# harvardinformatics/IMCoalHMM

Hardware: AMD Instinct MI355X
Metric: alignment columns/sec (forward pass), 20-state isolation HMM (higher is better)
Workload: dtype f64

## Files before the change

imcoalhmm_amd/csrc/imcoal_fwd.hip:

```cpp
#include <hip/hip_runtime.h>

#include <algorithm>
#include <array>
#include <cerrno>
#include <climits>
#include <cmath>
#include <cstdint>
#include <cstdio>
#include <cstdlib>
#include <cstring>
#include <list>
#include <atomic>
#include <chrono>
#include <map>
#include <set>
#include <memory>
#include <mutex>
#include <condition_variable>
#include <string>
#include <vector>

#include <sys/stat.h>
#include <unistd.h>

#include "../../include/imcoal_fwd.h"
#include "kernels_plain.hpp"
#include "kernels_stitch.hpp"
#include "kernels_zip.hpp"
#include "kernels_big.hpp"
#include "kernels_zip2.hpp"
#include "kernels_zip3.hpp"
#include "kernels_zip4.hpp"
#include "options_host.hpp"
#include "pair_dict.hpp"
#include "kernels_encode.hpp"
#include "kernels_train.hpp"
#include "kernels_ingest.hpp"
#include "kernels_align.hpp"
#include "kernels_phylip.hpp"
#include "slab_stream.hpp"
#include "plan_host.hpp"
#include "planner_host.hpp"
#include "model_host.hpp"
#include "kernels_model.hpp"
#include "../../include/imcoal_model.h"
#include "kernels_sample.hpp"
#include "../../include/imcoal_sample.h"
#include "obs_io.hpp"
#include "fasta_io.hpp"

static_assert(sizeof(imc::Desc4) == sizeof(int4) && alignof(imc::Desc4) == alignof(int4), "descriptor entries are uploaded as int4");

namespace {

thread_local std::string g_err;
std::mutex g_mu;
std::condition_variable g_cv;

int fail(int code, const std::string &msg)
{
    g_err = msg;
    return code;
}

#define HIP_TRY(expr)                                                                                   \
    do {                                                                                                \
        hipError_t _e = (expr);                                                                         \
        if (_e != hipSuccess)                                                                           \
            return fail(_e == hipErrorOutOfMemory ? IMC_ERR_OOM : IMC_ERR_HIP,                          \
                        std::string(#expr) + ": " + hipGetErrorString(_e));                             \
    } while (0)

using imc::HYBRID_MAX_ALPHABET;
using imc::LDS_BUDGET;
using imc::Z2GRAN;
using imc::round_up;

constexpr size_t STAGE_KERNEL_MAX_BYTES = 1u << 20;

struct GuardRec { hipDeviceptr_t va; size_t va_size; hipMemGenericAllocationHandle_t handle; hipDeviceptr_t map; size_t map_size; };
std::map<void *, GuardRec> &g_guard = *new std::map<void *, GuardRec>();

void dev_free(void *p)
{
    if (!p) return;
    auto it = g_guard.find(p);
    if (it == g_guard.end()) { (void)hipFree(p); return; }
    (void)hipDeviceSynchronize();
    (void)hipMemUnmap(it->second.map, it->second.map_size);
    (void)hipMemRelease(it->second.handle);
    g_guard.erase(it);
}

struct DictDev : imc::TrainedDict {
// ... 1525 lines not shown
        std::vector<std::pair<int, int>> table_runs;
        DevBuf<double> d_Cpack;
        bool rank1 = false;
        std::vector<int> checkpoints;
        std::vector<BigBlock> tail_blocks;
        std::vector<std::pair<uint32_t, uint32_t>> r1_segs;
        DevBuf<BigBlock> d_tail_blocks;
        DevBuf<int> d_r1flag, d_r1at;
        DevBuf<double> d_r1u, d_r1alpha;
    } chain;

    struct Blocked {
        std::vector<Z2Block> blocks;
        DevBuf<Z2Block> d_blocks;
        DevBuf<uint16_t> d_tab_order;
        DevBuf<int> d_tab_lvl;
        std::vector<int> tab_lvl;
        int tab_nlvl = 0;
        DevBuf<int4> d_tab_desc;
        DevBuf<int4> d_tab_desc2;
        std::vector<std::pair<int, int>> tab2;
        DevBuf<int4> d_tab_desc3;
        std::vector<std::pair<int, int>> tab3;
        bool wide_tokens = false;
        bool stream_table = false;
        int n_hot = 0;
        std::vector<uint16_t> hot;
        DevBuf<uint16_t> d_hot;
        imc::PhaseTable phases;
        std::vector<Z2Tail> tails;
        DevBuf<Z2Tail> d_tails;
        DevBuf<double> d_tailX;
        DevBuf<int> d_tailE, d_tail_arrive;
        int tail_stride = 0;
    } blk;
};

struct Level {
    uint32_t n_segs = 0, n_vecs = 0, n_chains = 0;
    DevBuf<uint32_t> d_vec0;
    DevBuf<uint8_t> d_first;
    DevBuf<ChainDesc> d_chains;
    DevBuf<double> d_P;
    DevBuf<int> d_EX, d_EMAX;
};

struct PlanKey {
    std::vector<uint64_t> chunk_ids;
    int N = 0, S = 0, B = 0;
    bool op_mode = false;
    imc::PlanOptions opt;
    bool operator==(const PlanKey &o) const
    {
        return chunk_ids == o.chunk_ids && N == o.N && S == o.S && B == o.B && op_mode == o.op_mode && opt.force_level == o.opt.force_level &&
               imc::same_plan_options(opt, o.opt);
    }
};

struct Plan {
    const PlanKey key;
    KernelChoice *kc = nullptr;
    bool wide = false;
    const int &N = key.N, &S = key.S, &B = key.B;
    const int n_chunks = (int)key.chunk_ids.size();
    uint32_t n_segs = 0, n_vecs = 0;
    std::vector<Group> groups;
    size_t pstride = 0;
    DevBuf<SegDesc> d_segs;
    DevBuf<VecDesc> d_vecs;
    std::vector<Level> levels;
    DevBuf<int32_t> d_final_vec;
    uint64_t chain_steps = 0;
    bool finish_fused = false;
    DevBuf<double> d_params, d_out;
    double *h_params[2] = {nullptr, nullptr};
    hipEvent_t ev_params[2] = {nullptr, nullptr};
    bool ev_used[2] = {false, false};
    int slot = 0;
    double *h_out = nullptr;
    double *h_out_dev = nullptr;
    double *h_params_dev[2] = {nullptr, nullptr};
    hipStream_t last_stream = nullptr;
    int last_slot = 0;
    bool have_last = false;
    bool busy = false;
    hipGraphExec_t graph = nullptr;
    uint64_t calls = 0;
    uint64_t lp[8] = {0, 0, 0, 0, 0, 0, 0, 0};
    std::string kernels;
    explicit Plan(PlanKey k) : key(std::move(k)) {}
    Plan(const Plan &) = delete;
    Plan &operator=(const Plan &) = delete;
    ~Plan()
    {
        if (graph) (void)hipGraphExecDestroy(graph);
        for (int k = 0; k < 2; ++k) {
            if (h_params[k]) (void)hipHostFree(h_params[k]);
            if (ev_params[k]) (void)hipEventDestroy(ev_params[k]);
        }
        if (h_out) (void)hipHostFree(h_out);
    }
};

std::list<std::unique_ptr<Plan>> &g_plans = *new std::list<std::unique_ptr<Plan>>();
constexpr size_t MAX_PLANS = 4;

void wait_all_idle(std::unique_lock<std::mutex> &lk)
// ... 100 lines not shown
void publish_last(const Plan *p)
{
    for (int k = 0; k < 8; ++k) g.last_plan[k] = p->lp[k];
    g.last_kernels = p->kernels;
}

struct DevUpload {
    hipError_t e = hipSuccess;
    template <class T> void alloc(DevBuf<T> &d, size_t bytes)
    {
        if (e == hipSuccess) e = d.alloc(std::max<size_t>(bytes, 16));
    }
    template <class T> void zeroed(DevBuf<T> &d, size_t bytes)
    {
        alloc(d, bytes);
        if (e == hipSuccess) e = hipMemset(d.get(), 0, std::max<size_t>(bytes, 16));
    }
    template <class T, class V> void put(DevBuf<T> &d, const std::vector<V> &h)
    {
        static_assert(sizeof(T) == sizeof(V), "the device buffer holds the host vector's elements");
        alloc(d, h.size() * sizeof(V));
        if (e == hipSuccess && !h.empty()) e = hipMemcpy(d.get(), h.data(), h.size() * sizeof(V), hipMemcpyHostToDevice);
    }
    template <class F> void then(F f)
    {
        if (e == hipSuccess) e = f();
    }
};

struct PlanBuilder {
    const imc_obs *const *chunks = nullptr;
    int n_chunks = 0, N = 0, S = 0, B = 0;
    bool op_mode = false;
    KernelChoice *kc = nullptr;
    bool wide = false;
    bool mfma() const { return kc->use3(opt().blocked_variant) || wide; }
    std::unique_ptr<Plan> p;
    const imc::PlanOptions &opt() const { return p->key.opt; }
    std::vector<int> chunk_group;
    std::vector<SegDesc> segs;
    std::vector<uint8_t> seg_first;
    std::vector<uint32_t> chunk_seg;
    std::vector<VecDesc> vecs;
    std::vector<std::vector<std::pair<uint32_t, uint32_t>>> chunk_units;
    std::vector<uint32_t> chunk_unit, unit_vec0;
    std::vector<uint8_t> unit_first;
    struct HostLevel { std::vector<uint32_t> chunk_seg, vec0; std::vector<uint8_t> first; std::vector<ChainDesc> chains; uint32_t n_vecs; };
    std::vector<HostLevel> hl;
    std::vector<int32_t> final_vec;

    void cut_segments()
    {
        chunk_seg.assign(n_chunks + 1, 0);
        for (int f = 0; f < n_chunks; ++f) {
            chunk_seg[f] = (uint32_t)segs.size();
            const Group &gr = p->groups[chunk_group[f]];
            const size_t L = gr.tokens ? chunks[f]->ntok[gr.level] : chunks[f]->L;
            const uint8_t *base = gr.tokens ? chunks[f]->d_tok[gr.level] : chunks[f]->d_sym;
            if (!L) continue;
            const size_t K0 = (L + gr.seglen - 1) / gr.seglen;
            const size_t sl = round_up((L + K0 - 1) / K0, gr.is_blocked() ? Z2GRAN : 16);
            for (size_t off = 0, k = 0; off < L; off += sl, ++k) {
                const bool wide = gr.tokens ? chunks[f]->wide[gr.level] : chunks[f]->wide_raw;
                const bool fst = k == 0 && !op_mode;
                segs.push_back(SegDesc{base + off * (wide ? 2 : 1), (uint32_t)std::min(sl, L - off),
                                       (fst ? SEG_FIRST : 0u) | (wide ? SEG_WIDE : 0u)});
                seg_first.push_back(fst);
            }
        }
        chunk_seg[n_chunks] = (uint32_t)segs.size();
    }

    int make_units()
    {
        chunk_units.assign(n_chunks, {});
        for (int f = 0; f < n_chunks; ++f) {
            const Group &gr = p->groups[chunk_group[f]];
            const uint32_t step = gr.is_blocked() ? (uint32_t)kc->z4_slots() : 1u;
            for (uint32_t sid = chunk_seg[f]; sid < chunk_seg[f + 1]; sid += step)
                chunk_units[f].push_back({sid, std::min(step, chunk_seg[f + 1] - sid)});
        }
        chunk_unit.assign(n_chunks + 1, 0);
        for (int f = 0; f < n_chunks; ++f) chunk_unit[f + 1] = chunk_unit[f] + (uint32_t)chunk_units[f].size();
        unit_vec0.assign(chunk_unit[n_chunks], 0);
        unit_first.assign(chunk_unit[n_chunks], 0);
        for (Group &gr : p->groups) {
            gr.vec_begin = (uint32_t)vecs.size();
            for (int f : gr.chunks) {
                gr.stream_len += gr.tokens ? chunks[f]->ntok[gr.level] : chunks[f]->L;
                for (size_t u = 0; u < chunk_units[f].size(); ++u) {
                    const uint32_t sid = chunk_units[f][u].first, ns = chunk_units[f][u].second;
                    const uint32_t uid = chunk_unit[f] + (uint32_t)u;
                    const bool fst = seg_first[sid] != 0;
                    unit_first[uid] = fst;
                    unit_vec0[uid] = (uint32_t)vecs.size();
                    const int nv = fst ? 1 : N;
                    for (int c = 0; c < nv; ++c) vecs.push_back(VecDesc{sid, (uint32_t)c});
                    if (gr.is_chain()) { gr.chain.seg_ids.push_back(sid); gr.chain.seg_out.push_back(unit_vec0[uid]); }
                    if (gr.is_blocked()) {
                        std::vector<Z2Block> &blocks = gr.blk.blocks;
                        const bool whole = mfma() && fst && ns == 1 && chunk_units[f].size() == 1;
                        if (whole && !blocks.empty() && blocks.back().first == 2 && blocks.back().n < (uint32_t)kc->z4_slots() &&
                            blocks.back().seg0 + blocks.back().n == sid && blocks.back().out_vec0 + blocks.back().n == unit_vec0[uid])
                            ++blocks.back().n;
                        else
                            blocks.push_back(Z2Block{sid, ns, unit_vec0[uid], whole ? 2u : fst ? 1u : 0u});
                    }
                    for (uint32_t q2 = 0; q2 < ns; ++q2)
                        gr.vsteps += (uint64_t)((seg_first[sid + q2] && !gr.is_blocked()) ? 1 : N) * segs[sid + q2].len;
                }
            }
            gr.n_vecs = (uint32_t)vecs.size() - gr.vec_begin;
        }
        if (p->groups.size() == 1 && p->groups[0].is_blocked() && mfma() && !op_mode && n_chunks > 0) {
            Group::Blocked &bl = p->groups[0].blk;
            bool ok = true;
            size_t most = 0;
            for (int f = 0; f < n_chunks; ++f) {
                ok = ok && !chunk_units[f].empty() && chunk_units[f].size() <= (size_t)kc->z4_slots();
// ... 165 lines not shown
                u.zeroed(ch.d_r1flag, nrec * 4);
                u.zeroed(ch.d_r1at, nrec * 4);
                u.alloc(ch.d_r1u, nrec * kc->NP * 8);
                u.alloc(ch.d_r1alpha, nrec * kc->NP * 8);
            }
        }
        u.alloc(q->d_params, (size_t)B * q->pstride * 8);
        u.alloc(q->d_out, (size_t)B * std::max(n_chunks, 1) * 8);
        for (int k = 0; k < 2; ++k) {
            u.then([&] { return hipHostMalloc((void **)&q->h_params[k], (size_t)B * q->pstride * 8, hipHostMallocMapped); });
            u.then([&] { return hipHostGetDevicePointer((void **)&q->h_params_dev[k], q->h_params[k], 0); });
            u.then([&] { return hipEventCreateWithFlags(&q->ev_params[k], hipEventDisableTiming); });
        }
        u.then([&] { return hipHostMalloc((void **)&q->h_out, (size_t)B * std::max(n_chunks, 1) * 8, hipHostMallocMapped); });
        u.then([&] { return hipHostGetDevicePointer((void **)&q->h_out_dev, q->h_out, 0); });
        if (u.e != hipSuccess)
            return fail(u.e == hipErrorOutOfMemory ? IMC_ERR_OOM : IMC_ERR_HIP,
                        std::string("plan allocation: ") + hipGetErrorString(u.e));
        g_plans.push_front(std::move(p));
        *out = q;
        return IMC_OK;
    }
};

void gather_facts(const imc_obs *const *chunks, int n_chunks, std::vector<imc::ChunkFacts> &cf, std::vector<imc::DictFacts> &df,
                  std::vector<std::shared_ptr<DictDev>> &dict_of)
{
    cf.resize(n_chunks);
    for (int f = 0; f < n_chunks; ++f) {
        const imc_obs *o = chunks[f];
        imc::ChunkFacts &c = cf[f];
        c.L = o->L; c.nsym = o->nsym; c.wide_raw = o->wide_raw;
        if (o->dict) {
            c.dict = (int)(std::find(dict_of.begin(), dict_of.end(), o->dict) - dict_of.begin());
            if (c.dict == (int)dict_of.size()) { dict_of.push_back(o->dict); df.push_back(imc::DictFacts{&o->dict->depth}); }
        }
        for (int l = 0; l < imc::kNumLevels; ++l)
            c.level[l] = imc::ChunkFacts::Level{o->d_tok[l] != nullptr, o->wide[l], o->ntok[l], o->alphabet[l], &o->tok_count[l]};
    }
}

int build_plan(const imc_obs *const *chunks, int n_chunks, int N, int S, int B, bool op_mode, Plan **out)
{
    PlanKey key;
    key.chunk_ids.reserve(n_chunks);
    for (int f = 0; f < n_chunks; ++f) key.chunk_ids.push_back(chunks[f]->id);
    key.N = N; key.S = S; key.B = B; key.op_mode = op_mode;
    static_cast<imc::Options &>(key.opt) = g.opt;
    key.opt.cus = g.cus;
    const char *force_level = std::getenv("IMC_FORCE_LEVEL");
    key.opt.force_level = force_level ? std::atoi(force_level) : -1;
    key.opt.debug = std::getenv("IMC_DEBUG") != nullptr;
    key.opt.debug_levels = std::getenv("IMC_DEBUG_LEVELS") != nullptr;
    const imc::PlanOptions &opt = key.opt;
    for (auto it = g_plans.begin(); it != g_plans.end(); ++it) {
        if ((*it)->key == key) {
            g_plans.splice(g_plans.begin(), g_plans, it);
            *out = g_plans.front().get();
            return IMC_OK;
        }
    }
    std::vector<imc::ChunkFacts> cf;
    std::vector<imc::DictFacts> df;
    std::vector<std::shared_ptr<DictDev>> dict_of;
    gather_facts(chunks, n_chunks, cf, df, dict_of);

    KernelChoice *kc = choose_kernel(N, imc::prefer_gemm(opt, cf, N, S));
    if (!kc) return fail(IMC_ERR_ARG, "N exceeds the largest built kernel (" + std::to_string(IMC_MAX_N) + ")");
    if (kc->R == 0 && (kc->G == 7 || kc->G == 9) && kc + 1 < kChoices + sizeof(kChoices) / sizeof(kChoices[0]) &&
        imc::next_shape_hands_off(opt, *kc, *(kc + 1), cf, S, B))
        kc = kc + 1;
    imc::PlanDecision dec = imc::decide_groups(opt, *kc, false, cf, df, N, S, B, op_mode);
    bool wide = false;
    KernelChoice *kw = (N > 24 && N <= 32) ? choose_kernel(N, false) : nullptr;
    if (kw && kw->wide_blocked && opt.wide_blocked != 0 && opt.compression == 1 && opt.kernel_pref == 0 && n_chunks > 0) {
        imc::PlanDecision wdec = imc::decide_groups(opt, *kw, true, cf, df, N, S, B, op_mode);
        if (imc::wide_plan_wins(opt, dec, kc->R == 0, wdec, cf, N)) {
            dec = std::move(wdec);
            kc = kw;
            wide = true;
        }
    }
    PlanBuilder pb;
    pb.chunks = chunks; pb.n_chunks = n_chunks; pb.N = N; pb.S = S; pb.B = B; pb.op_mode = op_mode; pb.kc = kc; pb.wide = wide;
    pb.p = std::make_unique<Plan>(std::move(key));
    pb.p->kc = kc; pb.p->wide = wide;
    pb.chunk_group = std::move(dec.chunk_group);
    for (imc::GroupDecision &gd : dec.groups) {
        Group gr;
        gr.kind = gd.kind; gr.tokens = gd.tokens; gr.level = gd.level; gr.A = gd.A;
        if (gd.dict >= 0) gr.dict = dict_of[gd.dict];
        gr.chunks = std::move(gd.chunks);
        gr.seglen = gd.seglen; gr.model_us = gd.model_us; gr.model_tab_us = gd.model_tab_us;
        gr.blk.wide_tokens = gd.wide_tokens;
        gr.chain.rank1 = gd.rank1; gr.chain.checkpoints = std::move(gd.checkpoints);
        pb.p->groups.push_back(std::move(gr));
    }
    pb.cut_segments();
    if (int rc = pb.make_units()) return rc;
    pb.make_hierarchy();
    return pb.upload(out);
}

int check_args(const imc_obs *const *chunks, int n_chunks, int B, int N, int S, const double *pis,
               const double *Ts, const double *Es)
{
// ... 237 lines not shown
                                   (const int4 *)gr.blk.d_tab_desc3.get(), lc.first, lc.second, staged);
            else
                hipLaunchKernelGGL(kc->zip4_level3, grid, dim3(Z4L3_WAVES * 64), kc->zip4_level3_lds(0), stream, ba,
                                   (const int4 *)gr.blk.d_tab_desc3.get(), lc.first, lc.second, none);
            head = false;
            HIP_TRY(hipGetLastError());
        }
    } else if (opt.table_pairs && gr.blk.d_tab_desc2 && kc->zip4_level2) {
        const size_t split_max = opt.table_split_max >= 0 ? (size_t)opt.table_split_max : (size_t)4 * opt.cus;
        for (const auto &lc : gr.blk.tab2) {
            if (opt.table_split && (size_t)lc.second * B <= split_max) {
                if (head)
                    hipLaunchKernelGGL(kc->zip4_level2_split_first, dim3((unsigned)(lc.second + Z4_SPLIT_WAVES_FIRST - 1) / Z4_SPLIT_WAVES_FIRST, (unsigned)B),
                                       dim3(Z4_SPLIT_WAVES_FIRST * 64), p->pstride * 8, stream, ba,
                                       (const int4 *)gr.blk.d_tab_desc2.get(), lc.first, lc.second, staged);
                else
                    hipLaunchKernelGGL(kc->zip4_level2_split, dim3((unsigned)(lc.second + Z4_SPLIT_WAVES - 1) / Z4_SPLIT_WAVES, (unsigned)B),
                                       dim3(Z4_SPLIT_WAVES * 64), 0, stream, ba,
                                       (const int4 *)gr.blk.d_tab_desc2.get(), lc.first, lc.second, none);
                split_used = true;
            } else if (head)
                hipLaunchKernelGGL(kc->zip4_level2_first, dim3((unsigned)(lc.second + 3) / 4, (unsigned)B), dim3(64),
                                   p->pstride * 8, stream, ba,
                                   (const int4 *)gr.blk.d_tab_desc2.get(), lc.first, lc.second, staged);
            else
                hipLaunchKernelGGL(kc->zip4_level2, dim3((unsigned)(lc.second + 3) / 4, (unsigned)B), dim3(64), 0, stream, ba,
                                   (const int4 *)gr.blk.d_tab_desc2.get(), lc.first, lc.second, none);
            head = false;
            HIP_TRY(hipGetLastError());
        }
    } else
        for (int d = 0; d < gr.blk.tab_nlvl; ++d) {
            const int first = gr.blk.tab_lvl[d], count = gr.blk.tab_lvl[d + 1] - first;
            hipLaunchKernelGGL(kc->zip4_level, dim3((unsigned)(count + 3) / 4, (unsigned)B), dim3(64), 0, stream, ba, first, count);
            HIP_TRY(hipGetLastError());
        }
    return IMC_OK;
}

int Launch::zip4(const Group &gr)
{
    BigArgs ba = blocked_args(gr);
    if (int rc = z4_table(gr, ba)) return rc;
    void (*scan)(BigArgs) = gr.blk.stream_table ? (gr.blk.wide_tokens ? kc->zip4sw : kc->zip4s) : (gr.blk.wide_tokens ? kc->zip4w : kc->zip4);
    if (int rc = allow_lds_budget(scan)) return rc;
    if (int rc = mark_a()) return rc;
    dim3 scan_grid(ba.n_group_segs, (unsigned)B);
    if (opt.xcd_affine && B > 1) {
        const imc::PhaseTable &t = gr.blk.phases;
        ba.n_phases = t.n_phases;
        for (int k = 0; k < t.n_phases; ++k) { ba.ph_begin[k] = t.ph_begin[k]; ba.ph_first[k] = t.ph_first[k]; ba.ph_sets[k] = t.ph_sets[k]; }
        scan_grid = dim3((unsigned)t.grid);
    }
    hipLaunchKernelGGL(scan, scan_grid, dim3(kc->z4_waves * 64), kc->zip4_lds(gr.A, gr.blk.n_hot), stream, ba);
    note(std::string("k_zpropagate4<") + std::to_string(kc->NP / 4) + (gr.blk.wide_tokens ? ",16" : "") + (gr.blk.stream_table ? ",streamed>" : ">") + stream_tag(gr));
    account(gr);
    HIP_TRY(hipGetLastError());
    return IMC_OK;
}

int Launch::zip32(const Group &gr)
{
    BigArgs ba = blocked_args(gr);
    const bool v3 = kc->use3(opt.blocked_variant);
    void (*scan)(BigArgs) = v3 ? kc->zip3 : kc->zip2;
    if (int rc = allow_lds_budget(scan)) return rc;
    size_t lds3 = kc->blocked_lds(gr.A, opt.blocked_variant);
    if (direct_params) { ba.params_src = p->h_params_dev[p->slot]; lds3 = ((lds3 + 15) & ~(size_t)15) + p->pstride * 8; }
    hipLaunchKernelGGL(scan, dim3(ba.n_group_segs, (unsigned)p->B), dim3(Z2WAVES * 64), lds3, stream, ba);
    note(std::string(v3 ? "k_zpropagate3<" : "k_zpropagate2<") + std::to_string(kc->NP / 4) + ">" + stream_tag(gr));
    account(gr);
    HIP_TRY(hipGetLastError());
    return IMC_OK;
}


int Launch::zpropagate(const Group &gr)
{
    const size_t lds = kc->zip_lds(gr.A);
    if (int rc = allow_lds_budget(kc->zip)) return rc;
    const uint32_t vpb = (uint32_t)(ZWAVES * kc->VPW);
    dim3 grid((gr.n_vecs + vpb - 1) / vpb, (unsigned)p->B);
    hipLaunchKernelGGL(kc->zip, grid, dim3(ZWAVES * 64), lds, stream, prop_args(p, gr));
    note("k_zpropagate<" + std::to_string(kc->R) + "," + std::to_string(kc->G) + ">" + stream_tag(gr));
    account(gr);
    HIP_TRY(hipGetLastError());
    return IMC_OK;
}

int Launch::propagate(const Group &gr)
{
    const uint32_t vpb = (uint32_t)(WPB * kc->VPW);
    dim3 grid((gr.n_vecs + vpb - 1) / vpb, (unsigned)p->B);
    const size_t lds = ((size_t)WPB * kc->VPW * kc->NP + (size_t)p->S * kc->NP) * 8;
    if (lds > LDS_BUDGET) return fail(IMC_ERR_ARG, "emission table (S x N) too large for LDS");
    if (lds > 48 * 1024)
        if (int rc = allow_lds_budget(kc->plain)) return rc;
    hipLaunchKernelGGL(kc->plain, grid, dim3(WPB * 64), lds, stream, prop_args(p, gr));
    note("k_propagate<" + std::to_string(kc->R) + "," + std::to_string(kc->G) + ">" + stream_tag(gr));
    account(gr);
    HIP_TRY(hipGetLastError());
    return IMC_OK;
}


int Launch::stitch() const
// ... 1315 lines not shown
```

imcoalhmm_amd/csrc/kernels_big.hpp:

```cpp
#pragma once
#include "kernels_plain.hpp"

typedef double v4f64 __attribute__((ext_vector_type(4)));

struct Z2Block {
    uint32_t seg0, n;
    uint32_t out_vec0;
    uint32_t first;
};

struct Z2Tail { uint32_t chunk, unit, n_units, pad; };

struct BigArgs {
    const SegDesc *segs;
    const uint32_t *seg_ids;
    const uint32_t *seg_vec0;
    const Z2Block *blocks;
    uint32_t n_group_segs;
    uint32_t n_vecs_total;
    int N, S, A;
    const double *params;
    const double *params_src;
    size_t pstride;
    int PP;
    const uint16_t *tok_left, *tok_right;
    double *Ctab;
    int *cex;
    double *P;
    int *EX;
    int phase;
    int t_from, t_to;
    int *r1flag;
    int *r1at;
    double *r1u, *r1alpha;
    uint32_t n_segs;
    const uint16_t *tab_order;
    const int *tab_lvl;
    int tab_nlvl;
    const uint16_t *hot;
    int n_hot;
    const int4 *tab_desc;
    double *Cpack;
    int TS;
    const Z2Tail *tail;
    double *tailX;
    int *tailE;
    int *tail_arrive;
    double *tail_out;
    int tail_stride, n_chunks;
    int n_phases, ph_begin[4], ph_first[4], ph_sets[4];
};


template <int NT>
struct BigLds {
    static constexpr int NP = 16 * NT;
    static constexpr int APS = 18;
    static constexpr int BPS = NP + 4;
    static constexpr int A_DOUBLES = NP * APS, B_DOUBLES = 16 * BPS;
    static constexpr size_t bytes = (size_t)2 * (A_DOUBLES + B_DOUBLES) * 8;
};

template <int NT, int TC = NT>
__device__ __forceinline__ void big_gemm(const double *__restrict__ A, const double *__restrict__ B, int row0, int col0,
                                         int tid, double *lds, v4f64 (&acc)[1][TC])
{
    using L = BigLds<NT>;
    constexpr int NP = 16 * NT, TR = 1, THREADS = NT * 64;
    constexpr int APS = L::APS, BPS = L::BPS;
    const int lane = tid & 63, lm = lane & 15, lg = lane >> 4;
    const int e0 = tid, e1 = tid + THREADS;
    const int ar0 = e0 >> 3, ac0 = e0 & 7, ar1 = e1 >> 3, ac1 = e1 & 7;
    const int br0 = e0 / (NP / 2), bc0 = e0 - br0 * (NP / 2), br1 = e1 / (NP / 2), bc1 = e1 - br1 * (NP / 2);
    const double *gA0 = A + (size_t)ar0 * NP + 2 * ac0, *gA1 = A + (size_t)ar1 * NP + 2 * ac1;
    const double *gB0 = B + (size_t)br0 * NP + 2 * bc0, *gB1 = B + (size_t)br1 * NP + 2 * bc1;
    const int lA0 = ar0 * APS + 2 * ac0, lA1 = ar1 * APS + 2 * ac1;
    const int lB0 = L::A_DOUBLES + br0 * BPS + 2 * bc0, lB1 = L::A_DOUBLES + br1 * BPS + 2 * bc1;
    double2 sa0, sa1, sb0, sb1;
#define BIG_FETCH(kb_)                                                                 \
    do {                                                                               \
        sa0 = *reinterpret_cast<const double2 *>(gA0 + (kb_) * 16);                    \
        sa1 = *reinterpret_cast<const double2 *>(gA1 + (kb_) * 16);                    \
        sb0 = *reinterpret_cast<const double2 *>(gB0 + (size_t)(kb_) * 16 * NP);       \
        sb1 = *reinterpret_cast<const double2 *>(gB1 + (size_t)(kb_) * 16 * NP);       \
    } while (0)
#define BIG_STAGE(buf_)                                                                \
    do {                                                                               \
        double *base_ = lds + (buf_) * (L::A_DOUBLES + L::B_DOUBLES);                  \
        *reinterpret_cast<double2 *>(base_ + lA0) = sa0;                               \
        *reinterpret_cast<double2 *>(base_ + lA1) = sa1;                               \
        *reinterpret_cast<double2 *>(base_ + lB0) = sb0;                               \
        *reinterpret_cast<double2 *>(base_ + lB1) = sb1;                               \
    } while (0)
#pragma unroll
    for (int tr = 0; tr < TR; ++tr)
#pragma unroll
        for (int tc = 0; tc < TC; ++tc) acc[tr][tc] = v4f64{0.0, 0.0, 0.0, 0.0};
    BIG_FETCH(0);
    BIG_STAGE(0);
    __syncthreads();
#pragma unroll 1
    for (int kb = 0; kb < NP / 16; ++kb) {
        const int buf = kb & 1;
// ... 828 lines not shown
```

imcoalhmm_amd/csrc/kernels_zip4.hpp:

```cpp
#pragma once
#include "kernels_zip3.hpp"

template <int NT>
struct Zip4Shape {
    static constexpr int WAVES = NT <= 6 ? Z2WAVES : 4;
    static constexpr int SLOTS = WAVES * 4;
    static constexpr bool SLOT_MAP = NT <= 6;
};

template <int NT>
struct Zip4Geom {
    using G3 = Zip3Geom<NT>;
    static constexpr int TOK = G3::TOK;
    static constexpr int SLOTS = Zip4Shape<NT>::SLOTS;
    static constexpr int MAPS = Zip4Shape<NT>::SLOT_MAP ? 2 : 1;
    static constexpr int slots(int H) { return (H + 1 > SLOTS + 1 ? H + 1 : SLOTS + 1); }
    static constexpr size_t lds_bytes(int A, int H) { return (size_t)slots(H) * TOK * 8 + (size_t)(MAPS * (A + 2) + 64) * 4 + 16; }
    static constexpr int max_hot(int A, size_t budget)
    {
        const size_t fixed = (size_t)(MAPS * (A + 2) + 64) * 4 + 16;
        const size_t n = budget > fixed ? (budget - fixed) / ((size_t)TOK * 8) : 0;
        return n > 1 ? (int)n - 1 : 0;
    }
};
// ... 543 lines not shown
    const double *Gt = a.Ctab + (size_t)b * (a.A + 1) * TOK;
    const int *Gc = a.cex + (size_t)b * (a.A + 1);
    const int IDENT = a.A;
    const double *Gi = Gt + (size_t)IDENT * TOK;

    Z4_STAMP(0);
    for (int z = tid; z <= a.A; z += THREADS) { cex[z] = Gc[z]; if constexpr (SLOT_MAP) slot_of[z] = -1; }
    if constexpr (HYB) {
        __syncthreads();
        for (int k = tid; k <= H; k += THREADS) slot_of[k < H ? (int)a.hot[k] : IDENT] = k;
        for (int idx = tid; idx < (H + 1) * (TOK / 2); idx += THREADS) {
            const int k = idx / (TOK / 2), w = idx - k * (TOK / 2);
            const int z = k < H ? (int)a.hot[k] : IDENT;
            reinterpret_cast<double2 *>(C + (size_t)k * TOK)[w] = reinterpret_cast<const double2 *>(Gt + (size_t)z * TOK)[w];
        }
    }
    __syncthreads();

    Z4_STAMP(1);
    const int lane = tid & 63;
    const int q = lane >> 4, bq = (lane >> 2) & 3, r = lane & 3;
    const int lo = (q * 4 + r) * Geo::NTE, lx = q * 4 + r;
    const Z2Block blk = a.blocks[bx];
    const int slot = (tid >> 6) * 4 + bq;
    const bool valid = slot < (int)blk.n;
    const uint32_t seg = blk.seg0 + (valid ? slot : ((slot & ~3) < (int)blk.n ? (slot & ~3) : 0));
    const SegDesc sd = a.segs[seg];
    const int len = valid ? (int)sd.len : 0;
    const bool first = (sd.first & SEG_FIRST) != 0;
    const uint8_t *tokp = sd.obs;
    typedef const __attribute__((address_space(1))) uint8_t *gptr;
    typedef uint32_t u32x4 __attribute__((ext_vector_type(4)));
    typedef const __attribute__((address_space(1))) u32x4 *gptr4;
    typedef const __attribute__((address_space(1))) uint32_t *gptr1;
    const gptr tokg = (gptr)tokp;

    double P[NT][NT], Q[NT][NT];
    {
        const int tok0 = (valid && first) ? seg_token(tokp, WIDE, 0) : 0;
#pragma unroll
        for (int K = 0; K < NT; ++K)
#pragma unroll
            for (int J = 0; J < NT; ++J) {
                const int i = 4 * K + q, c = 4 * J + r;
                double v;
                if (first) v = (c == 0 && i < a.N) ? pi_p[i] * Etg[(size_t)tok0 * a.PP + i] : 0.0;
                else v = (i == c && i < a.N) ? 1.0 : 0.0;
                P[K][J] = valid ? v : 0.0;
            }
    }
    int ex = 0;
    const int maxlen = wave_max_i32(len);
    const int nfull = maxlen == 0 ? 0 : wave_min_i32(valid ? len / RESCALE_EVERY : INT_MAX);

    constexpr int RING = (!HYB && NT <= 4) ? 2 : 1;
    constexpr int ROWS = NT == 8 ? 4 : NT;
    double al[NT] = {}, pre[RING][ROWS][NT];
#pragma unroll
    for (int d = 0; d < RING; ++d)
#pragma unroll
        for (int I = 0; I < ROWS; ++I)
#pragma unroll
            for (int K = 0; K < NT; ++K) pre[d][I][K] = 0.0;
    auto mk = [&](int tok) __attribute__((always_inline)) {
        Z4Tok t;
        t.s = HYB ? slot_of[tok] : -1;
        t.ce = cex[tok];
        t.tok = tok;
        return t;
    };
    auto prime = [&](const Z4Tok &c, const Z4Tok &c1) __attribute__((always_inline)) {
        if constexpr (HYB) zip3_load_row<NT>(al, C + (size_t)max(c.s, 0) * TOK, 0, lo, lx);
        const double *Gc0 = c.s < 0 ? Gt + (size_t)c.tok * TOK : Gi;
#pragma unroll
        for (int I = 0; I < ROWS; ++I) zip4_load_row_global<NT>(pre[0][I], Gc0, I, lo, lx);
        if constexpr (RING == 2) {
            const double *Gc1 = Gt + (size_t)c1.tok * TOK;
#pragma unroll
            for (int I = 0; I < ROWS; ++I) zip4_load_row_global<NT>(pre[1][I], Gc1, I, lo, lx);
        }
    };
    auto two_steps = [&](const Z4Tok &t0, const Z4Tok &t1, const Z4Tok &tn, const Z4Tok &tn1) __attribute__((always_inline)) {
        if constexpr (RING == 2) {
            zip4_step<NT, HYB, ROWS>(P, Q, C, Gt, Gi, t0, t1, tn, al, pre[0], lo, lx);
            zip4_step<NT, HYB, ROWS>(Q, P, C, Gt, Gi, t1, tn, tn1, al, pre[1], lo, lx);
        } else {
            zip4_step<NT, HYB, ROWS>(P, Q, C, Gt, Gi, t0, t1, t1, al, pre[0], lo, lx);
            zip4_step<NT, HYB, ROWS>(Q, P, C, Gt, Gi, t1, tn, tn, al, pre[0], lo, lx);
        }
        ex += t0.ce + t1.ce;
    };
    constexpr int PER = WIDE ? 8 : 16;
    auto masked_run = [&](int bi, int u0, int n) __attribute__((always_inline)) {
        uint4 ob = make_uint4(0u, 0u, 0u, 0u);
        if (bi * RESCALE_EVERY + u0 < len) {
            const u32x4 v = *(gptr4)(tokg + ((size_t)bi * RESCALE_EVERY + u0) * TB);
            ob = make_uint4(v.x, v.y, v.z, v.w);
        }
        const int live = len - bi * RESCALE_EVERY - u0;
        const int dead0 = (first && bi == 0 && u0 == 0) ? 0 : -1;
        const unsigned long long lo64 = (unsigned long long)ob.y << 32 | ob.x, hi64 = (unsigned long long)ob.w << 32 | ob.z;
        auto tok_of = [&](int v) __attribute__((always_inline)) {
            const unsigned long long h = v < PER / 2 ? lo64 : hi64;
            const int tk = WIDE ? (int)((h >> (16 * (v & 3))) & 0xffffull) : (int)((h >> (8 * (v & 7))) & 0xffull);
            return (v < live && v != dead0 && v < PER) ? tk : IDENT;
        };
        Z4Tok c0 = mk(tok_of(0)), c1 = mk(tok_of(1));
        prime(c0, c1);
#pragma unroll 1
        for (int v = 0; v < n; v += 2) {
            const Z4Tok c2 = mk(tok_of(v + 2)), c3 = mk(tok_of(v + 3));
            two_steps(c0, c1, c2, c3);
            c0 = c2;
            c1 = c3;
        }
    };
    auto masked_block = [&](int bi, int npos) __attribute__((always_inline)) {
#pragma unroll 1
        for (int u0 = 0; u0 < npos; u0 += PER) masked_run(bi, u0, min(PER, npos - u0));
        zip3_rescale<NT>(P, ex);
    };
    if (nfull == 0 && maxlen > 0) masked_block(0, min(RESCALE_EVERY, (maxlen + 1) & ~1));
    Z4_STAMP(2);
    if (nfull > 0) {
        constexpr int NW = 4 * TB;
        constexpr uint32_t TM = WIDE ? 0xffffu : 0xffu;
        auto load_words = [&](int bi, uint32_t (&w)[NW]) __attribute__((always_inline)) {
            gptr4 src = (gptr4)(tokg + (size_t)bi * RESCALE_EVERY * TB);
            const u32x4 x = src[0];
            w[0] = x.x; w[1] = x.y; w[2] = x.z; w[3] = x.w;
            if constexpr (WIDE) {
                const u32x4 y = src[1];
                w[4] = y.x; w[5] = y.y; w[6] = y.z; w[7] = y.w;
            }
        };
        uint32_t cw[NW];
        load_words(0, cw);
        Z4Tok c0 = mk(first ? IDENT : (int)(cw[0] & TM));
        prime(c0, mk(WIDE ? (int)(cw[0] >> 16) : (int)((cw[0] >> 8) & TM)));
        for (int bi = 0; bi < nfull; ++bi) {
            const bool more = bi + 1 < nfull;
            const int bn = more ? bi + 1 : bi;
            const uint32_t nfirst = *(gptr1)(tokg + (size_t)bn * RESCALE_EVERY * TB);
#pragma unroll
            for (int g4 = 0; g4 < 4; ++g4) {
                int t1, t2, t3, t4;
                if constexpr (WIDE) {
                    const uint32_t wa = cw[0], wb = cw[1];
#pragma unroll
                    for (int k = 0; k + 2 < NW; ++k) cw[k] = cw[k + 2];
                    t1 = (int)(wa >> 16); t2 = (int)(wb & TM); t3 = (int)(wb >> 16);
                } else {
                    const uint32_t wa = cw[0];
#pragma unroll
                    for (int k = 0; k + 1 < NW; ++k) cw[k] = cw[k + 1];
                    t1 = (int)((wa >> 8) & TM); t2 = (int)((wa >> 16) & TM); t3 = (int)(wa >> 24);
                }
                t4 = g4 < 3 ? (int)(cw[0] & TM) : more ? (int)(nfirst & TM) : IDENT;
                const uint32_t w5 = g4 < 3 ? cw[0] : nfirst;
                const int t5 = (g4 < 3 || more) ? (WIDE ? (int)(w5 >> 16) : (int)((w5 >> 8) & TM)) : IDENT;
                if (g4 == 3) load_words(bn, cw);
                const Z4Tok c1 = mk(t1), c2 = mk(t2), c3 = mk(t3);
                two_steps(c0, c1, c2, c3);
                const Z4Tok c4 = mk(t4), c5 = mk(t5);
                two_steps(c2, c3, c4, c5);
                c0 = c4;
            }
            zip3_rescale<NT>(P, ex);
        }
    }
    Z4_STAMP(3);
    for (int bi = max(1, nfull); bi * RESCALE_EVERY < maxlen; ++bi)
        masked_block(bi, min(RESCALE_EVERY, (maxlen - bi * RESCALE_EVERY + 1) & ~1));
    zip3_rescale<NT>(P, ex);
    Z4_STAMP(4);
#ifdef IMC_Z4_TIMING
    if ((threadIdx.x & 63) == 0 && blockIdx.x < 1024 && blockIdx.y == 0) g_z4_dbg[1024 * 8 + blockIdx.x * 8 + (threadIdx.x >> 6)] = wall_clock64();
#endif

    if (blk.first == 2) {
        if (valid && r == 0) {
            const size_t gvp = (size_t)b * a.n_vecs_total + blk.out_vec0 + slot;
#pragma unroll
            for (int K = 0; K < NT; ++K)
                if (4 * K + q < a.N) a.P[gvp * NP + 4 * K + q] = P[K][0];
            if (q == 0) a.EX[gvp] = ex;
        }
        return;
    }

    zip3_fold<NT, HYB, true, SLOTS>(P, ex, C, xex, (int)blk.n, slot, tid >> 6, lo, lx);

    Z4_STAMP(5);
#ifdef IMC_Z4_TIMING
    if (threadIdx.x == 0 && blockIdx.x < 1024 && blockIdx.y == 0) g_z4_dbg[blockIdx.x * 8 + 7] = (long long)nfull * 1000000 + maxlen;
#endif
    if (slot == 0) {
        const size_t gv = (size_t)b * a.n_vecs_total + blk.out_vec0;
        double *Pout = a.P + gv * NP;
        if (blk.first) {
            if (r == 0) {
#pragma unroll
                for (int K = 0; K < NT; ++K)
                    if (4 * K + q < a.N) Pout[4 * K + q] = P[K][0];
            }
            if (q == 0 && r == 0) a.EX[gv] = ex;
        } else {
#pragma unroll
            for (int K = 0; K < NT; ++K)
#pragma unroll
                for (int J = 0; J < NT; ++J) {
                    const int i = 4 * K + q, c = 4 * J + r;
                    if (i < a.N && c < a.N) Pout[(size_t)i * NP + c] = P[K][J];
                }
            if (q == 0) {
#pragma unroll
                for (int J = 0; J < NT; ++J)
                    if (4 * J + r < a.N) a.EX[gv + 4 * J + r] = ex;
            }
        }
    }
    if (a.tail) zip3_tail<NT, SLOTS>(a, P, ex, C, xex, b, bx, slot, lo, lx);
}
```

imcoalhmm_amd/csrc/planner_host.hpp:

```cpp
#pragma once

#include <algorithm>
#include <cmath>
#include <cstddef>
#include <cstdint>
#include <cstdio>
#include <functional>
#include <map>
#include <set>
#include <utility>
#include <vector>

#include "options_host.hpp"
#include "pair_dict.hpp"
#include "plan_host.hpp"

namespace imc {

constexpr double Z4_STREAM_MAX_BYTES = 32.0e6;
constexpr size_t LDS_BUDGET = 160 * 1024 - 1024;
constexpr size_t CTAB_BUDGET = (size_t)24 << 30;
#ifndef IMC_HYBRID_MAX_ALPHABET
#define IMC_HYBRID_MAX_ALPHABET 4096
#endif
constexpr int HYBRID_MAX_ALPHABET = IMC_HYBRID_MAX_ALPHABET;
constexpr size_t Z2GRAN = 4;
constexpr size_t R1_MIN_SEGLEN = 1024;
constexpr size_t R1_MIN_HEAD = 256;
constexpr double R1_HEAD_COLUMNS = 65536.0;
constexpr double R1_HEAD_MIN_COLUMNS = 8192.0;
constexpr int R1_MAX_ROUNDS = 24;
constexpr double R1_DENSE_COLUMNS = 1.0e5;

enum class GroupKind {
    ColumnVector,
    TokenVector,
    BlockedLds,
    BlockedGlobal,
    GemmChain,
    MatVecChain,
};

struct PlanOptions : Options {
    int cus = 256;
    int force_level = -1;
    bool debug = false;
    bool debug_levels = false;
};

struct KernelFacts {
    int R = 0, G = 0, NP = 0, VPW = 0, minw = 1;
    int zwaves = 0;
    int big_nslab = 0;
    size_t big_lds = 0;
    int tok_doubles = 0;
    int z4_waves = 8;
    bool wide_blocked = false;
    bool has_zip2 = false, has_zip3 = false, has_zip4 = false, has_zip4s = false, has_level2 = false;
    size_t (*zip_lds)(int) = nullptr;
    size_t (*zip2_lds)(int) = nullptr;
    size_t (*zip3_lds)(int) = nullptr;
    size_t (*zip4_lds)(int, int) = nullptr;
    int (*zip4_max_hot)(int, size_t) = nullptr;
    int z4_slots() const { return z4_waves * 4; }
    bool use3(int blocked_variant) const { return has_zip3 && blocked_variant >= 3; }
    size_t blocked_lds(int A, int blocked_variant) const { return use3(blocked_variant) ? zip3_lds(A) : zip2_lds(A); }
};

struct ChunkFacts {
    size_t L = 0;
    int nsym = 0;
    bool wide_raw = false;
    int dict = -1;
    struct Level {
        bool stream = false;
        bool wide = false;
        size_t ntok = 0;
        int alphabet = 0;
        const std::vector<uint32_t> *tok_count = nullptr;
        const std::vector<uint32_t> &counts() const
        {
            static const std::vector<uint32_t> none;
            return tok_count ? *tok_count : none;
        }
    } level[kNumLevels];
};

struct DictFacts {
    const std::vector<int> *depth = nullptr;
};

struct GroupDecision {
    bool tokens = false;
    int level = -1, A = 0;
    int dict = -1;
    std::vector<int> chunks;
    GroupKind kind = GroupKind::ColumnVector;
    size_t seglen = 0;
    bool wide_tokens = false;
    bool rank1 = false;
// ... 482 lines not shown
```

Before: 400.2 billion.

## Balance segment cuts across CUs and pipeline the uniform tail block in zip4

Adds a host-side balanced cutter that uses spare workgroup slots in the last dispatch round to split long chunks into more, shorter segments. Within each workgroup it alternates two segment lengths across the slot halves. In the zip4 scan kernel, when every lane shares the same length and the remainder after the full rescale blocks is even, the tail is run as a pipelined continuation of the token stream instead of the masked block path. Both are on by default and can be turned off with environment variables. The risks are uneven per-lane lengths breaking the uniform-length assumption, and extra segment joins adding stitch work.

```diff
diff --git a/imcoalhmm_amd/csrc/cut_host.hpp b/imcoalhmm_amd/csrc/cut_host.hpp
--- /dev/null
+++ b/imcoalhmm_amd/csrc/cut_host.hpp
@@ -0,0 +1,79 @@
+#pragma once
+
+#include <algorithm>
+#include <cstddef>
+#include <cstdint>
+#include <vector>
+
+namespace imc {
+
+struct ChunkCut {
+    uint32_t a = 0, b = 0;
+    uint32_t workgroups = 0;
+    bool balanced = false;
+};
+
+inline size_t equal_seglen(size_t L, size_t seglen, size_t gran)
+{
+    const size_t K0 = (L + seglen - 1) / seglen;
+    return ((L + K0 - 1) / K0 + gran - 1) / gran * gran;
+}
+
+inline void cut_lengths(const ChunkCut &c, size_t L, int slots, std::vector<uint32_t> &out)
+{
+    out.clear();
+    for (size_t off = 0, k = 0; off < L; ++k) {
+        const size_t len = std::min<size_t>((int)(k % (size_t)slots) < slots / 2 ? c.a : c.b, L - off);
+        out.push_back((uint32_t)len);
+        off += len;
+    }
+}
+
+inline std::vector<ChunkCut> balanced_cut(const std::vector<size_t> &tokens, size_t seglen, int slots, int B, int cus, size_t gran,
+                                          size_t keep_within = 0)
+{
+    const size_t n = tokens.size(), half = (size_t)slots / 2;
+    std::vector<ChunkCut> cut(n);
+    std::vector<size_t> W(n, 0);
+    size_t total = 0, run = 0;
+    for (size_t f = 0; f < n; ++f) {
+        const size_t L = tokens[f];
+        if (!L) continue;
+        const size_t sl = equal_seglen(L, seglen, gran), nseg = (L + sl - 1) / sl;
+        cut[f].a = cut[f].b = (uint32_t)sl;
+        W[f] = (nseg + slots - 1) / slots;
+        cut[f].workgroups = (uint32_t)W[f];
+        if (nseg == 1) { if (run++ % (size_t)slots == 0) ++total; }
+        else { run = 0; total += W[f]; }
+    }
+    if (B < 1 || cus < 1 || half == 0 || slots % 2) return cut;
+    auto sum_len = [&](size_t L, size_t w) { return ((L + half * w - 1) / (half * w) + gran - 1) / gran * gran; };
+    const size_t wgs = total * (size_t)B, rounds = (wgs + cus - 1) / (size_t)cus;
+    std::vector<size_t> Wn = W;
+    for (size_t spare = (rounds * (size_t)cus - wgs) / (size_t)B; spare > 0; --spare) {
+        size_t best = n;
+        for (size_t f = 0; f < n; ++f) {
+            if (W[f] < 2 || sum_len(tokens[f], Wn[f] + 1) < 32) continue;
+            if (W[f] <= keep_within && Wn[f] + 1 > keep_within) continue;
+            if (best == n || tokens[f] * Wn[best] > tokens[best] * Wn[f]) best = f;
+        }
+        if (best == n) break;
+        ++Wn[best];
+    }
+    for (size_t f = 0; f < n; ++f) {
+        if (W[f] < 2) continue;
+        const size_t L = tokens[f], T = sum_len(L, Wn[f]);
+        if (T < 32) continue;
+        size_t a = T / 2 / 16 * 16;
+        if (a < 16 || T - 2 * a >= 16) a = T / 2 / gran * gran;
+        const size_t b = T - a;
+        if (a == b && (Wn[f] == W[f] || a == cut[f].a)) continue;
+        cut[f].a = (uint32_t)a;
+        cut[f].b = (uint32_t)b;
+        cut[f].workgroups = (uint32_t)((L + half * T - 1) / (half * T));
+        cut[f].balanced = true;
+    }
+    return cut;
+}
+
+}
diff --git a/imcoalhmm_amd/csrc/imcoal_fwd.hip b/imcoalhmm_amd/csrc/imcoal_fwd.hip
--- a/imcoalhmm_amd/csrc/imcoal_fwd.hip
+++ b/imcoalhmm_amd/csrc/imcoal_fwd.hip
@@ -40,6 +40,7 @@
 #include "kernels_phylip.hpp"
 #include "slab_stream.hpp"
 #include "plan_host.hpp"
+#include "cut_host.hpp"
 #include "planner_host.hpp"
 #include "model_host.hpp"
 #include "kernels_model.hpp"
@@ -1671,7 +1672,7 @@
     imc::PlanOptions opt;
     bool operator==(const PlanKey &o) const
     {
-        return chunk_ids == o.chunk_ids && N == o.N && S == o.S && B == o.B && op_mode == o.op_mode && opt.force_level == o.opt.force_level &&
+        return chunk_ids == o.chunk_ids && N == o.N && S == o.S && B == o.B && op_mode == o.op_mode && opt.force_level == o.opt.force_level && opt.balanced_cut == o.opt.balanced_cut && opt.tail_pipe == o.opt.tail_pipe &&
                imc::same_plan_options(opt, o.opt);
     }
 };
@@ -1878,19 +1879,37 @@
     void cut_segments()
     {
         chunk_seg.assign(n_chunks + 1, 0);
+        auto stream_len = [&](int f) { const Group &gr = p->groups[chunk_group[f]]; return gr.tokens ? chunks[f]->ntok[gr.level] : chunks[f]->L; };
+        std::vector<imc::ChunkCut> balanced(n_chunks);
+        for (const Group &gr : p->groups) {
+            if (!opt().balanced_cut || !gr.global_table() || wide || kc->z4_waves != 8 || op_mode || opt().seg_override) continue;
+            std::vector<size_t> lens;
+            bool packs = false;
+            for (int f : gr.chunks) {
+                lens.push_back(stream_len(f));
+                packs = packs || (lens.back() && lens.back() <= imc::equal_seglen(lens.back(), gr.seglen, Z2GRAN));
+            }
+            if (packs && p->groups.size() > 1) continue;
+            const size_t keep = opt().fuse_tail == 0 ? 0 : opt().fuse_tail == 2 ? (size_t)kc->z4_slots() : 4;
+            const std::vector<imc::ChunkCut> cut = imc::balanced_cut(lens, gr.seglen, kc->z4_slots(), B, opt().cus, Z2GRAN, keep);
+            for (size_t k = 0; k < gr.chunks.size(); ++k) balanced[gr.chunks[k]] = cut[k];
+        }
+        std::vector<uint32_t> lens;
         for (int f = 0; f < n_chunks; ++f) {
             chunk_seg[f] = (uint32_t)segs.size();
             const Group &gr = p->groups[chunk_group[f]];
-            const size_t L = gr.tokens ? chunks[f]->ntok[gr.level] : chunks[f]->L;
+            const size_t L = stream_len(f);
             const uint8_t *base = gr.tokens ? chunks[f]->d_tok[gr.level] : chunks[f]->d_sym;
             if (!L) continue;
-            const size_t K0 = (L + gr.seglen - 1) / gr.seglen;
-            const size_t sl = round_up((L + K0 - 1) / K0, gr.is_blocked() ? Z2GRAN : 16);
-            for (size_t off = 0, k = 0; off < L; off += sl, ++k) {
+            imc::ChunkCut cut = balanced[f];
+            if (!cut.balanced)
+                cut.a = cut.b = (uint32_t)imc::equal_seglen(L, gr.seglen, gr.is_blocked() ? Z2GRAN : 16);
+            imc::cut_lengths(cut, L, kc->z4_slots(), lens);
+            size_t off = 0;
+            for (size_t k = 0; k < lens.size(); off += lens[k], ++k) {
                 const bool wide = gr.tokens ? chunks[f]->wide[gr.level] : chunks[f]->wide_raw;
                 const bool fst = k == 0 && !op_mode;
-                segs.push_back(SegDesc{base + off * (wide ? 2 : 1), (uint32_t)std::min(sl, L - off),
-                                       (fst ? SEG_FIRST : 0u) | (wide ? SEG_WIDE : 0u)});
+                segs.push_back(SegDesc{base + off * (wide ? 2 : 1), lens[k], (fst ? SEG_FIRST : 0u) | (wide ? SEG_WIDE : 0u)});
                 seg_first.push_back(fst);
             }
         }
@@ -2162,6 +2181,10 @@
     key.opt.force_level = force_level ? std::atoi(force_level) : -1;
     key.opt.debug = std::getenv("IMC_DEBUG") != nullptr;
     key.opt.debug_levels = std::getenv("IMC_DEBUG_LEVELS") != nullptr;
+    const char *balanced_cut = std::getenv("IMC_BALANCED_CUT");
+    key.opt.balanced_cut = !balanced_cut || std::atoi(balanced_cut) != 0;
+    const char *tail_pipe = std::getenv("IMC_TAIL_PIPE");
+    key.opt.tail_pipe = !tail_pipe || std::atoi(tail_pipe) != 0;
     const imc::PlanOptions &opt = key.opt;
     for (auto it = g_plans.begin(); it != g_plans.end(); ++it) {
         if ((*it)->key == key) {
@@ -2505,6 +2528,7 @@
         for (int k = 0; k < t.n_phases; ++k) { ba.ph_begin[k] = t.ph_begin[k]; ba.ph_first[k] = t.ph_first[k]; ba.ph_sets[k] = t.ph_sets[k]; }
         scan_grid = dim3((unsigned)t.grid);
     }
+    ba.z4_tail_pipe = opt.tail_pipe ? 1 : 0;
     hipLaunchKernelGGL(scan, scan_grid, dim3(kc->z4_waves * 64), kc->zip4_lds(gr.A, gr.blk.n_hot), stream, ba);
     note(std::string("k_zpropagate4<") + std::to_string(kc->NP / 4) + (gr.blk.wide_tokens ? ",16" : "") + (gr.blk.stream_table ? ",streamed>" : ">") + stream_tag(gr));
     account(gr);
diff --git a/imcoalhmm_amd/csrc/kernels_big.hpp b/imcoalhmm_amd/csrc/kernels_big.hpp
--- a/imcoalhmm_amd/csrc/kernels_big.hpp
+++ b/imcoalhmm_amd/csrc/kernels_big.hpp
@@ -49,6 +49,7 @@
     double *tail_out;
     int tail_stride, n_chunks;
     int n_phases, ph_begin[4], ph_first[4], ph_sets[4];
+    int z4_tail_pipe;
 };
 
 
diff --git a/imcoalhmm_amd/csrc/kernels_zip4.hpp b/imcoalhmm_amd/csrc/kernels_zip4.hpp
--- a/imcoalhmm_amd/csrc/kernels_zip4.hpp
+++ b/imcoalhmm_amd/csrc/kernels_zip4.hpp
@@ -619,6 +619,8 @@
     int ex = 0;
     const int maxlen = wave_max_i32(len);
     const int nfull = maxlen == 0 ? 0 : wave_min_i32(valid ? len / RESCALE_EVERY : INT_MAX);
+    const int rem = maxlen - nfull * RESCALE_EVERY;
+    const bool piped = a.z4_tail_pipe != 0 && nfull > 0 && rem > 0 && (rem & 1) == 0 && wave_min_i32(valid ? len : INT_MAX) == maxlen;
 
     constexpr int RING = (!HYB && NT <= 4) ? 2 : 1;
     constexpr int ROWS = NT == 8 ? 4 : NT;
@@ -692,21 +694,21 @@
     if (nfull > 0) {
         constexpr int NW = 4 * TB;
         constexpr uint32_t TM = WIDE ? 0xffffu : 0xffu;
-        auto load_words = [&](int bi, uint32_t (&w)[NW]) __attribute__((always_inline)) {
+        auto load_words = [&](int bi, uint32_t (&w)[NW], bool second) __attribute__((always_inline)) {
             gptr4 src = (gptr4)(tokg + (size_t)bi * RESCALE_EVERY * TB);
             const u32x4 x = src[0];
             w[0] = x.x; w[1] = x.y; w[2] = x.z; w[3] = x.w;
             if constexpr (WIDE) {
-                const u32x4 y = src[1];
+                const u32x4 y = src[second ? 1 : 0];
                 w[4] = y.x; w[5] = y.y; w[6] = y.z; w[7] = y.w;
             }
         };
         uint32_t cw[NW];
-        load_words(0, cw);
+        load_words(0, cw, true);
         Z4Tok c0 = mk(first ? IDENT : (int)(cw[0] & TM));
         prime(c0, mk(WIDE ? (int)(cw[0] >> 16) : (int)((cw[0] >> 8) & TM)));
         for (int bi = 0; bi < nfull; ++bi) {
-            const bool more = bi + 1 < nfull;
+            const bool more = bi + 1 < nfull || piped;
             const int bn = more ? bi + 1 : bi;
             const uint32_t nfirst = *(gptr1)(tokg + (size_t)bn * RESCALE_EVERY * TB);
 #pragma unroll
@@ -726,7 +728,7 @@
                 t4 = g4 < 3 ? (int)(cw[0] & TM) : more ? (int)(nfirst & TM) : IDENT;
                 const uint32_t w5 = g4 < 3 ? cw[0] : nfirst;
                 const int t5 = (g4 < 3 || more) ? (WIDE ? (int)(w5 >> 16) : (int)((w5 >> 8) & TM)) : IDENT;
-                if (g4 == 3) load_words(bn, cw);
+                if (g4 == 3) load_words(bn, cw, bi + 1 < nfull || !piped || rem > 8);
                 const Z4Tok c1 = mk(t1), c2 = mk(t2), c3 = mk(t3);
                 two_steps(c0, c1, c2, c3);
                 const Z4Tok c4 = mk(t4), c5 = mk(t5);
@@ -735,9 +737,29 @@
             }
             zip3_rescale<NT>(P, ex);
         }
+        if (piped) {
+#pragma unroll 1
+            for (int v = 0; v < rem; v += 2) {
+                int t1, t2, t3;
+                if constexpr (WIDE) {
+                    t1 = (int)(cw[0] >> 16); t2 = (int)(cw[1] & TM); t3 = (int)(cw[1] >> 16);
+#pragma unroll
+                    for (int k = 0; k + 1 < NW; ++k) cw[k] = cw[k + 1];
+                } else {
+                    t1 = (int)((cw[0] >> 8) & TM); t2 = (int)((cw[0] >> 16) & TM); t3 = (int)(cw[0] >> 24);
+#pragma unroll
+                    for (int k = 0; k + 1 < NW; ++k) cw[k] = cw[k] >> 16 | cw[k + 1] << 16;
+                    cw[NW - 1] >>= 16;
+                }
+                const Z4Tok c1 = mk(t1), c2 = mk(v + 2 < rem ? t2 : IDENT), c3 = mk(v + 3 < rem ? t3 : IDENT);
+                two_steps(c0, c1, c2, c3);
+                c0 = c2;
+            }
+            zip3_rescale<NT>(P, ex);
+        }
     }
     Z4_STAMP(3);
-    for (int bi = max(1, nfull); bi * RESCALE_EVERY < maxlen; ++bi)
+    for (int bi = piped ? INT_MAX / RESCALE_EVERY : max(1, nfull); bi * RESCALE_EVERY < maxlen; ++bi)
         masked_block(bi, min(RESCALE_EVERY, (maxlen - bi * RESCALE_EVERY + 1) & ~1));
     zip3_rescale<NT>(P, ex);
     Z4_STAMP(4);
diff --git a/imcoalhmm_amd/csrc/planner_host.hpp b/imcoalhmm_amd/csrc/planner_host.hpp
--- a/imcoalhmm_amd/csrc/planner_host.hpp
+++ b/imcoalhmm_amd/csrc/planner_host.hpp
@@ -46,6 +46,8 @@
     int force_level = -1;
     bool debug = false;
     bool debug_levels = false;
+    bool balanced_cut = true;
+    bool tail_pipe = true;
 };
 
 struct KernelFacts {
```

Result: no change. 401.9 billion, median of 2 (+0.4%).
